# Ham3798/shielded-pool-pinocchio-solana

Hardware: AMD Instinct MI355X
Metric: Groth16 proofs/sec (higher is better)
Workload: dtype u32x8 (254-bit Montgomery integers); 1 GPU; audit_circuit (RLWE, const-PK; scripts/generate_audit.py:246-465), batch of 2048 independent proofs per GPU per step, every row a distinct witness; circuit=audit, n_constraints=29178, n_wires=35432, domain=32768, batch_per_gpu=2048, n_distinct_witnesses=2048, table_bytes=226725433344, parallelism=independent proofs x1, pk_bytes=9850060

## Files before the change

shielded-pool-pinocchio-solana_amd/csrc/bn254_consts.hpp:

```cpp
#pragma once
#include <stdint.h>
namespace spp {
struct FrParams {
  static constexpr uint32_t MOD(int i) { constexpr uint32_t v[8] = {0xf0000001u, 0x43e1f593u, 0x79b97091u, 0x2833e848u, 0x8181585du, 0xb85045b6u, 0xe131a029u, 0x30644e72u}; return v[i]; }
  static constexpr uint32_t ONE(int i) { constexpr uint32_t v[8] = {0x4ffffffbu, 0xac96341cu, 0x9f60cd29u, 0x36fc7695u, 0x7879462eu, 0x666ea36fu, 0x9a07df2fu, 0x0e0a77c1u}; return v[i]; }
  static constexpr uint32_t R2(int i) { constexpr uint32_t v[8] = {0xae216da7u, 0x1bb8e645u, 0xe35c59e3u, 0x53fe3ab1u, 0x53bb8085u, 0x8c49833du, 0x7f4e44a5u, 0x0216d0b1u}; return v[i]; }
  static constexpr uint32_t R3(int i) { constexpr uint32_t v[8] = {0xb4bf0040u, 0x5e94d8e1u, 0x1cfbb6b8u, 0x2a489cbeu, 0xa19fcfedu, 0x893cc664u, 0x7fcc657cu, 0x0cf8594bu}; return v[i]; }
  static constexpr uint32_t HALF(int i) { constexpr uint32_t v[8] = {0xf8000000u, 0xa1f0fac9u, 0x3cdcb848u, 0x9419f424u, 0x40c0ac2eu, 0xdc2822dbu, 0x7098d014u, 0x18322739u}; return v[i]; }
  static constexpr uint32_t MODM2(int i) { constexpr uint32_t v[8] = {0xefffffffu, 0x43e1f593u, 0x79b97091u, 0x2833e848u, 0x8181585du, 0xb85045b6u, 0xe131a029u, 0x30644e72u}; return v[i]; }
  static constexpr uint32_t TWOP(int i) { constexpr uint32_t v[8] = {0xe0000002u, 0x87c3eb27u, 0xf372e122u, 0x5067d090u, 0x0302b0bau, 0x70a08b6du, 0xc2634053u, 0x60c89ce5u}; return v[i]; }
  static constexpr uint32_t INV32 = 0xefffffffu;
  static constexpr uint32_t K29_IN(int i) { constexpr uint32_t v[9] = {0x0fffead7u, 0x1d5444f4u, 0x04438aa5u, 0x03b4d096u, 0x134c84dau, 0x0e92d304u, 0x14cb95b3u, 0x041b9d3du, 0x00058003u}; return v[i]; }
  static constexpr uint32_t K29_ZZ_OUT(int i) { constexpr uint32_t v[9] = {0x00000000u, 0x00000000u, 0x00000000u, 0x00000000u, 0x00000000u, 0x00000000u, 0x00000000u, 0x00000000u, 0x00080000u}; return v[i]; }
  static constexpr uint32_t K29_ONE(int i) { constexpr uint32_t v[9] = {0x0fffff57u, 0x1ea70ab4u, 0x052c068bu, 0x17504f49u, 0x0aa8075bu, 0x1d4240ceu, 0x11d54c07u, 0x052ac7a8u, 0x000dc836u}; return v[i]; }
  static constexpr uint32_t SUBC_2P_1(int i) { constexpr uint32_t v[9] = {0x20000002u, 0x3e1f593eu, 0x3cb848a0u, 0x2fa121e5u, 0x2b0ba505u, 0x25b68180u, 0x214dc281u, 0x3cb84c67u, 0x0060c89bu}; return v[i]; }
  static constexpr uint32_t SUBC_4P_1(int i) { constexpr uint32_t v[9] = {0x20000004u, 0x3c3eb27du, 0x39709142u, 0x3f4243ccu, 0x36174a0bu, 0x2b6d0301u, 0x229b8503u, 0x397098cfu, 0x00c19138u}; return v[i]; }
  static constexpr uint32_t SUBC_6P_1(int i) { constexpr uint32_t v[9] = {0x20000006u, 0x3a5e0bbcu, 0x3628d9e4u, 0x2ee365b3u, 0x2122ef12u, 0x31238483u, 0x23e94785u, 0x3628e537u, 0x012259d5u}; return v[i]; }
  static constexpr uint32_t SUBC_8P_1(int i) { constexpr uint32_t v[9] = {0x20000008u, 0x387d64fbu, 0x32e12286u, 0x3e84879au, 0x2c2e9418u, 0x36da0604u, 0x25370a07u, 0x32e1319fu, 0x01832272u}; return v[i]; }
  static constexpr uint32_t SUBC_4P_3(int i) { constexpr uint32_t v[9] = {0x60000004u, 0x7c3eb27bu, 0x79709140u, 0x7f4243cau, 0x76174a09u, 0x6b6d02ffu, 0x629b8501u, 0x797098cdu, 0x00c19136u}; return v[i]; }
  static constexpr uint32_t SUBC_8P_3(int i) { constexpr uint32_t v[9] = {0x60000008u, 0x787d64f9u, 0x72e12284u, 0x7e848798u, 0x6c2e9416u, 0x76da0602u, 0x65370a05u, 0x72e1319du, 0x01832270u}; return v[i]; }
  static constexpr uint32_t SUBC_16P_3(int i) { constexpr uint32_t v[9] = {0x60000010u, 0x70fac9f5u, 0x65c2450cu, 0x7d090f34u, 0x785d2830u, 0x6db40c07u, 0x6a6e140eu, 0x65c2633du, 0x030644e4u}; return v[i]; }
};
struct FqParams {
  static constexpr uint32_t MOD(int i) { constexpr uint32_t v[8] = {0xd87cfd47u, 0x3c208c16u, 0x6871ca8du, 0x97816a91u, 0x8181585du, 0xb85045b6u, 0xe131a029u, 0x30644e72u}; return v[i]; }
  static constexpr uint32_t ONE(int i) { constexpr uint32_t v[8] = {0xc58f0d9du, 0xd35d438du, 0xf5c70b3du, 0x0a78eb28u, 0x7879462cu, 0x666ea36fu, 0x9a07df2fu, 0x0e0a77c1u}; return v[i]; }
  static constexpr uint32_t R2(int i) { constexpr uint32_t v[8] = {0x538afa89u, 0xf32cfc5bu, 0xd44501fbu, 0xb5e71911u, 0x0a417ff6u, 0x47ab1effu, 0xcab8351fu, 0x06d89f71u}; return v[i]; }
  static constexpr uint32_t R3(int i) { constexpr uint32_t v[8] = {0xda1530dfu, 0xb1cd6dafu, 0xa7283db6u, 0x62f210e6u, 0x0ada0afbu, 0xef7f0b0cu, 0x2d592544u, 0x20fd6e90u}; return v[i]; }
  static constexpr uint32_t HALF(int i) { constexpr uint32_t v[8] = {0x6c3e7ea3u, 0x9e10460bu, 0xb438e546u, 0xcbc0b548u, 0x40c0ac2eu, 0xdc2822dbu, 0x7098d014u, 0x18322739u}; return v[i]; }
  static constexpr uint32_t MODM2(int i) { constexpr uint32_t v[8] = {0xd87cfd45u, 0x3c208c16u, 0x6871ca8du, 0x97816a91u, 0x8181585du, 0xb85045b6u, 0xe131a029u, 0x30644e72u}; return v[i]; }
  static constexpr uint32_t TWOP(int i) { constexpr uint32_t v[8] = {0xb0f9fa8eu, 0x7841182du, 0xd0e3951au, 0x2f02d522u, 0x0302b0bbu, 0x70a08b6du, 0xc2634053u, 0x60c89ce5u}; return v[i]; }
  static constexpr uint32_t INV32 = 0xe4866389u;
  static constexpr uint32_t K29_IN(int i) { constexpr uint32_t v[9] = {0x13349ca1u, 0x1a5d84a8u, 0x0a3e5cacu, 0x100249e0u, 0x12b951e8u, 0x0e92d304u, 0x14cb95b3u, 0x041b9d3du, 0x00058003u}; return v[i]; }
  static constexpr uint32_t K29_ZZ_OUT(int i) { constexpr uint32_t v[9] = {0x00000000u, 0x00000000u, 0x00000000u, 0x00000000u, 0x00000000u, 0x00000000u, 0x00000000u, 0x00000000u, 0x00080000u}; return v[i]; }
  static constexpr uint32_t K29_ONE(int i) { constexpr uint32_t v[9] = {0x157ccc21u, 0x141c2758u, 0x185230d3u, 0x014c0419u, 0x0aa36fb9u, 0x1d4240ceu, 0x11d54c07u, 0x052ac7a8u, 0x000dc836u}; return v[i]; }
  static constexpr uint32_t SUBC_2P_1(int i) { constexpr uint32_t v[9] = {0x30f9fa8eu, 0x2208c16cu, 0x38e5469du, 0x25aa45a0u, 0x2b0bb2efu, 0x25b68180u, 0x214dc281u, 0x3cb84c67u, 0x0060c89bu}; return v[i]; }
  static constexpr uint32_t SUBC_4P_1(int i) { constexpr uint32_t v[9] = {0x21f3f51cu, 0x241182dau, 0x31ca8d3bu, 0x2b548b42u, 0x361765dfu, 0x2b6d0301u, 0x229b8503u, 0x397098cfu, 0x00c19138u}; return v[i]; }
  static constexpr uint32_t SUBC_6P_1(int i) { constexpr uint32_t v[9] = {0x32edefaau, 0x261a4447u, 0x2aafd3d9u, 0x30fed0e4u, 0x212318cfu, 0x31238483u, 0x23e94785u, 0x3628e537u, 0x012259d5u}; return v[i]; }
  static constexpr uint32_t SUBC_8P_1(int i) { constexpr uint32_t v[9] = {0x23e7ea38u, 0x282305b5u, 0x23951a77u, 0x36a91686u, 0x2c2ecbbfu, 0x36da0604u, 0x25370a07u, 0x32e1319fu, 0x01832272u}; return v[i]; }
  static constexpr uint32_t SUBC_4P_3(int i) { constexpr uint32_t v[9] = {0x61f3f51cu, 0x641182d8u, 0x71ca8d39u, 0x6b548b40u, 0x761765ddu, 0x6b6d02ffu, 0x629b8501u, 0x797098cdu, 0x00c19136u}; return v[i]; }
  static constexpr uint32_t SUBC_8P_3(int i) { constexpr uint32_t v[9] = {0x63e7ea38u, 0x682305b3u, 0x63951a75u, 0x76a91684u, 0x6c2ecbbdu, 0x76da0602u, 0x65370a05u, 0x72e1319du, 0x01832270u}; return v[i]; }
  static constexpr uint32_t SUBC_16P_3(int i) { constexpr uint32_t v[9] = {0x67cfd470u, 0x70460b69u, 0x672a34edu, 0x6d522d0bu, 0x785d977eu, 0x6db40c07u, 0x6a6e140eu, 0x65c2633du, 0x030644e4u}; return v[i]; }
};
}
```

shielded-pool-pinocchio-solana_amd/csrc/f29.hpp:

```cpp
#pragma once
#include "bn254.hpp"

#if defined(__HIPCC__)
#define SPP_HD_COLD __host__ __device__ __attribute__((noinline))
#else
#define SPP_HD_COLD __attribute__((noinline))
#endif

namespace spp {

template <class Pm>
struct F29 {
  uint32_t l[9];
  using Base = Fp<Pm>;
  typedef uint32_t (*ConstFn)(int);
  static constexpr uint32_t M = (1u << 29) - 1u;
  static constexpr uint32_t INV = Pm::INV32 & M;
  static SPP_HD constexpr uint32_t P9(int k) { return Base::P9(k); }

  template <ConstFn C>
  static SPP_HD F29 konst() {
    F29 r;
    SPP_UNROLL for (int i = 0; i < 9; i++) r.l[i] = C(i);
    return r;
// ... 62 lines not shown
  }
  SPP_HD F29 sqr() const {
    uint64_t c[18];
    clear(c);
    mac_sqr(c, *this);
    return reduce(c);
  }
  static SPP_HD F29 mul2(const F29& a, const F29& b, const F29& cc, const F29& d) {
    uint64_t c[18];
    clear(c);
    mac(c, a, b);
    mac(c, cc, d);
    return reduce(c);
  }

  template <ConstFn C>
  static SPP_HD F29 sub_lazy(const F29& a, const F29& b) {
    F29 r;
    SPP_UNROLL for (int k = 0; k < 9; k++) r.l[k] = a.l[k] + (C(k) - b.l[k]);
    return r;
  }
  template <ConstFn C>
  static SPP_HD F29 neg_lazy(const F29& b) {
    F29 r;
    SPP_UNROLL for (int k = 0; k < 9; k++) r.l[k] = C(k) - b.l[k];
    return r;
  }
  template <ConstFn C>
  static SPP_HD F29 sub_norm(const F29& a, const F29& b) {
    F29 r;
// ... 25 lines not shown
  }
  friend SPP_HD F29 add_norm(const F29& a, const F29& b) {
    F29 r;
    uint32_t carry = 0;
    SPP_UNROLL for (int k = 0; k < 8; k++) {
      const uint32_t t = a.l[k] + b.l[k] + carry;
      r.l[k] = t & M;
      carry = t >> 29;
    }
    r.l[8] = a.l[8] + b.l[8] + carry;
    return r;
  }

  template <uint32_t KMAX>
  SPP_HD bool is_zero_mod_p() const {
    uint32_t kk = 0xffffffffu;
    SPP_UNROLL for (uint32_t k = 0; k <= KMAX; k++) {
      if (l[0] == ((k * P9(0)) & M)) kk = k;
    }
    if (kk == 0xffffffffu) return false;
    uint32_t diff = 0, carry = 0;
    SPP_UNROLL for (int i = 0; i < 8; i++) {
      const uint32_t t = kk * P9(i) + carry;
      diff |= l[i] ^ (t & M);
      carry = t >> 29;
    }
    diff |= l[8] ^ (kk * P9(8) + carry);
    return diff == 0;
  }

  static SPP_HD F29 from_fp(const Base& a) { return from_words(a.l) * konst<Pm::K29_IN>(); }
  SPP_HD Base to_fp() const {
    uint32_t w[8];
    SPP_UNROLL for (int i = 0; i < 8; i++) w[i] = Pm::ONE(i);
    const F29 t = *this * from_words(w);
    Base r;
    t.to_words(r.l);
    return r;
  }
  SPP_HD Base scaled_to_fp() const {
    const F29 t = *this * konst<Pm::K29_ZZ_OUT>();
    Base r;
    t.to_words(r.l);
    return r;
  }
};

template <class Pm>
struct XYZZ29 {
  using F = F29<Pm>;
  using B = Fp<Pm>;
  F X, Y, ZZ, ZZZ;
  bool inf;

  static SPP_HD XYZZ29 infinity() {
    XYZZ29 r;
    SPP_UNROLL for (int i = 0; i < 9; i++) r.X.l[i] = r.Y.l[i] = r.ZZ.l[i] = r.ZZZ.l[i] = 0;
    r.inf = true;
    return r;
  }
  SPP_HD XYZZ<B> to_xyzz() const {
    if (inf) return XYZZ<B>::infinity();
    return {X.to_fp(), Y.to_fp(), ZZ.scaled_to_fp(), ZZZ.scaled_to_fp()};
// ... 11 lines not shown
  SPP_HD void madd(const Affine<B>& e, bool negate) { madd_any<false>(e, negate); }
  SPP_HD bool madd_distinct(const Affine<B>& e, bool negate) { return madd_any<true>(e, negate); }
  template <bool DISTINCT>
  SPP_HD bool madd_any(const Affine<B>& e, bool negate) {
    F x2 = F::from_words(e.x.l);
    F y2 = F::from_words(e.y.l);
    if (negate) y2 = F::template neg_lazy<Pm::SUBC_4P_1>(y2);
    if (inf) {
      X = x2 * F::template konst<Pm::K29_IN>();
      Y = y2 * F::template konst<Pm::K29_IN>();
      ZZ = F::template konst<Pm::K29_IN>();
      ZZZ = ZZ;
      inf = false;
      return true;
    }
    const F U2 = x2 * ZZ;
    const F Pp = F::template sub_norm<Pm::SUBC_6P_1>(U2, X);
    if (Pp.template is_zero_mod_p<7>()) {
      if constexpr (DISTINCT) return false;
      const F S2 = y2 * ZZZ;
      const F Rr = F::template sub_norm<Pm::SUBC_2P_1>(S2, Y);
      if (Rr.template is_zero_mod_p<3>()) {
        XYZZ<B> t = to_xyzz();
        t.dbl_inplace();
        const XYZZ29 d = from_xyzz(t);
        X = d.X;
        Y = d.Y;
        ZZ = d.ZZ;
        ZZZ = d.ZZZ;
      } else {
        inf = true;
      }
      return true;
    }
    const F PP = Pp.sqr();
    const F Q = X * PP;
    const F PPP = Pp * PP;
    ZZ = ZZ * PP;
    const F S2 = y2 * ZZZ;
    const F Rr = F::template sub_norm<Pm::SUBC_2P_1>(S2, Y);
    ZZZ = ZZZ * PPP;
    const F R2 = Rr.sqr();
    X = F::template sub3_norm<Pm::SUBC_4P_3>(R2, PPP, Q);
    const F T = F::template sub_lazy<Pm::SUBC_6P_1>(Q, X);
    const F Yn = F::template neg_lazy<Pm::SUBC_2P_1>(Y);
    Y = F::mul2(Rr, T, Yn, PPP);
    return true;
  }
};

struct F29x2 {
  using F = F29<FqParams>;
  using Pm = FqParams;
  F c0, c1;

  static SPP_HD F29x2 from_words(const Fq2& a) { return {F::from_words(a.c0.l), F::from_words(a.c1.l)}; }
  template <F::ConstFn CA>
  static SPP_HD F29x2 mul(const F29x2& a, const F29x2& b) {
    const F na1 = F::template neg_lazy<CA>(a.c1);
    return {F::mul2(a.c0, b.c0, na1, b.c1), F::mul2(a.c0, b.c1, a.c1, b.c0)};
  }
  SPP_HD F29x2 mul_real(const F& k) const { return {c0 * k, c1 * k}; }
  template <F::ConstFn CA>
  SPP_HD F29x2 sqr() const {
    const F s = add_lazy(c0, c1);
    const F d = F::template sub_lazy<CA>(c0, c1);
    const F t = add_lazy(c0, c0);
    return {s * d, t * c1};
  }
  template <F::ConstFn C>
  static SPP_HD F29x2 sub_norm(const F29x2& a, const F29x2& b) {
    return {F::template sub_norm<C>(a.c0, b.c0), F::template sub_norm<C>(a.c1, b.c1)};
  }
  template <F::ConstFn C>
  static SPP_HD F29x2 sub3_norm(const F29x2& a, const F29x2& b, const F29x2& c2) {
    return {F::template sub3_norm<C>(a.c0, b.c0, c2.c0), F::template sub3_norm<C>(a.c1, b.c1, c2.c1)};
  }
  template <F::ConstFn C>
  static SPP_HD F29x2 neg_lazy(const F29x2& a) {
    return {F::template neg_lazy<C>(a.c0), F::template neg_lazy<C>(a.c1)};
  }
  template <uint32_t KMAX>
  SPP_HD bool is_zero_mod_p() const {
    return c0.template is_zero_mod_p<KMAX>() && c1.template is_zero_mod_p<KMAX>();
  }
  SPP_HD Fq2 to_fp() const { return {c0.to_fp(), c1.to_fp()}; }
  SPP_HD Fq2 scaled_to_fp() const { return {c0.scaled_to_fp(), c1.scaled_to_fp()}; }
  static SPP_HD F29x2 from_fp(const Fq2& a) { return {F::from_fp(a.c0), F::from_fp(a.c1)}; }
};

struct XYZZ29G2 {
  using E = F29x2;
  using F = F29<FqParams>;
  using Pm = FqParams;
  E X, Y, ZZ, ZZZ;
  bool inf;

  static SPP_HD XYZZ29G2 infinity() {
    XYZZ29G2 r;
    SPP_UNROLL for (int i = 0; i < 9; i++) {
      r.X.c0.l[i] = r.X.c1.l[i] = r.Y.c0.l[i] = r.Y.c1.l[i] = 0;
      r.ZZ.c0.l[i] = r.ZZ.c1.l[i] = r.ZZZ.c0.l[i] = r.ZZZ.c1.l[i] = 0;
    }
    r.inf = true;
    return r;
  }
  SPP_HD XYZZ<Fq2> to_xyzz() const {
    if (inf) return XYZZ<Fq2>::infinity();
    return {X.to_fp(), Y.to_fp(), ZZ.scaled_to_fp(), ZZZ.scaled_to_fp()};
  }
  static SPP_HD XYZZ29G2 from_xyzz(const XYZZ<Fq2>& q) {
    XYZZ29G2 r;
    r.inf = q.is_inf();
    const F k = F::template konst<Pm::K29_IN>();
    r.X = E::from_fp(q.X);
    r.Y = E::from_fp(q.Y);
    r.ZZ = E::from_fp(q.ZZ).mul_real(k);
    r.ZZZ = E::from_fp(q.ZZZ).mul_real(k);
    return r;
  }

  SPP_HD void madd(const Affine<Fq2>& e, bool negate) { madd_any<false>(e, negate); }
  SPP_HD bool madd_distinct(const Affine<Fq2>& e, bool negate) { return madd_any<true>(e, negate); }
  template <bool DISTINCT>
  SPP_HD bool madd_any(const Affine<Fq2>& e, bool negate) {
    const E x2 = E::from_words(e.x);
    const E y2 = E::from_words(e.y);
// ... 3 lines not shown
      const E yn = E::template neg_lazy<Pm::SUBC_4P_1>(y2);
      E ys;
      SPP_UNROLL for (int i = 0; i < 9; i++) {
        ys.c0.l[i] = negate ? yn.c0.l[i] : y2.c0.l[i];
        ys.c1.l[i] = negate ? yn.c1.l[i] : y2.c1.l[i];
      }
      Y = ys.mul_real(k);
      SPP_UNROLL for (int i = 0; i < 9; i++) {
        ZZ.c0.l[i] = k.l[i];
        ZZ.c1.l[i] = 0;
      }
      ZZZ = ZZ;
      inf = false;
      return true;
    }
    const E U2 = E::template mul<Pm::SUBC_4P_1>(x2, ZZ);
    const E Pp = E::template sub_norm<Pm::SUBC_6P_1>(U2, X);
    E S2 = E::template mul<Pm::SUBC_4P_1>(y2, ZZZ);
    if (negate) S2 = E::template neg_lazy<Pm::SUBC_2P_1>(S2);
    const E Rr = E::template sub_norm<Pm::SUBC_2P_1>(S2, Y);
    if (Pp.template is_zero_mod_p<7>()) {
      if constexpr (DISTINCT) return false;
      if (Rr.template is_zero_mod_p<4>()) {
        XYZZ<Fq2> t = to_xyzz();
        t.dbl_inplace();
        const XYZZ29G2 d = from_xyzz(t);
        X = d.X;
        Y = d.Y;
        ZZ = d.ZZ;
        ZZZ = d.ZZZ;
      } else {
        inf = true;
      }
      return true;
    }
    const E PP = Pp.template sqr<Pm::SUBC_8P_1>();
    const E Q = E::template mul<Pm::SUBC_6P_1>(X, PP);
    const E PPP = E::template mul<Pm::SUBC_8P_1>(Pp, PP);
    ZZ = E::template mul<Pm::SUBC_2P_1>(ZZ, PP);
    ZZZ = E::template mul<Pm::SUBC_2P_1>(ZZZ, PPP);
    const E R2 = Rr.template sqr<Pm::SUBC_6P_1>();
    X = E::template sub3_norm<Pm::SUBC_4P_3>(R2, PPP, Q);
    const E T = E::template sub_norm<Pm::SUBC_6P_1>(Q, X);
    const F nR1 = F::template neg_lazy<Pm::SUBC_6P_1>(Rr.c1);
    const F nY0 = F::template neg_lazy<Pm::SUBC_2P_1>(Y.c0);
    const F nY1 = F::template neg_lazy<Pm::SUBC_2P_1>(Y.c1);
    uint64_t c[18];
    F::clear(c);
    F::mac(c, Rr.c0, T.c0);
    F::mac(c, nR1, T.c1);
    F::mac(c, nY0, PPP.c0);
    F::mac(c, Y.c1, PPP.c1);
    const F y0 = F::reduce(c);
    F::clear(c);
    F::mac(c, Rr.c0, T.c1);
    F::mac(c, Rr.c1, T.c0);
    F::mac(c, nY0, PPP.c1);
    F::mac(c, nY1, PPP.c0);
    Y.c0 = y0;
    Y.c1 = F::reduce(c);
    return true;
  }
};

}
```

shielded-pool-pinocchio-solana_amd/csrc/gen_consts.py:

```python
#!/usr/bin/env python3
R_MOD = 21888242871839275222246405745257275088548364400416034343698204186575808495617
Q_MOD = 21888242871839275222246405745257275088696311157297823662689037894645226208583


def limbs(v):
    return ", ".join("0x%08xu" % ((v >> (32 * i)) & 0xFFFFFFFF) for i in range(8))


def limbs29(v):
    return ", ".join("0x%08xu" % ((v >> (29 * i)) & ((1 << 29) - 1) if i < 8 else v >> 232) for i in range(9))


def lifted(m, k, lowmin):
    v = k * m
    c = [(v >> (29 * i)) & ((1 << 29) - 1) for i in range(8)] + [v >> 232]
    for i in range(8):
        while c[i] < lowmin:
            c[i] += 1 << 29
            c[i + 1] -= 1
    assert c[8] > 0 and sum(x << (29 * i) for i, x in enumerate(c)) == v and all(x < (1 << 32) for x in c)
    return c


def emit(name, m):
    W = 1 << 256
    inv32 = (-pow(m, -1, 1 << 32)) % (1 << 32)
    out = []
    out.append("struct %s {" % name)
    for cname, val in (("MOD", m), ("ONE", W % m), ("R2", W * W % m), ("R3", W * W * W % m),
                       ("HALF", (m - 1) // 2), ("MODM2", m - 2), ("TWOP", 2 * m)):
        out.append("  static constexpr uint32_t %s(int i) { constexpr uint32_t v[8] = {%s}; return v[i]; }"
                   % (cname, limbs(val)))
    out.append("  static constexpr uint32_t INV32 = 0x%08xu;" % inv32)
    W9 = 1 << 261
    for cname, val in (("K29_IN", W9 * W9 * pow(W, -1, m) % m),
                       ("K29_ZZ_OUT", W * W * pow(W9, -1, m) % m),
                       ("K29_ONE", W9 % m)):
        out.append("  static constexpr uint32_t %s(int i) { constexpr uint32_t v[9] = {%s}; return v[i]; }"
                   % (cname, limbs29(val)))
    for k, low in ((2, 1), (4, 1), (6, 1), (8, 1), (4, 3), (8, 3), (16, 3)):
        out.append("  static constexpr uint32_t SUBC_%dP_%d(int i) { constexpr uint32_t v[9] = {%s}; return v[i]; }"
                   % (k, low, ", ".join("0x%08xu" % x for x in lifted(m, k, low * ((1 << 29) - 1)))))
    out.append("};")
    return "\n".join(out)


print("// AUTO-GENERATED by gen_consts.py -- do not edit.")
print("#pragma once\n#include <stdint.h>\nnamespace spp {")
# ... 4 lines not shown
```

shielded-pool-pinocchio-solana_amd/csrc/kernels.hpp:

```cpp
#pragma once
#include <hip/hip_runtime.h>
#include <stdint.h>
#include "bn254.hpp"
#include "msm_plan.hpp"
#include "msm_ragged.hpp"
#include "rlwe_ntt.hpp"

namespace spp {

struct DevSparse {
  const uint32_t* rowptr;
  const uint32_t* wire;
  const uint32_t* coeff;
  const uint32_t* lit;
};
static constexpr uint32_t COEFF_ONE = 0x80000000u;
static constexpr uint32_t COEFF_MINUS_ONE = 0x40000000u;
static constexpr uint32_t COEFF_MASK = 0x3fffffffu;

struct HashConsts {
  const Fr* pos3_rc;  const Fr* pos3_mds;
  const Fr* pos5_rc;  const Fr* pos5_mds;
  const Fr* p2_rc;    const Fr* p2_mu;
  const uint32_t* pos3_mds29;
// ... 134 lines not shown
                         const int32_t* prov, const int32_t* proof_ok, int32_t dup, int32_t* result);
void launch_pool_commit(hipStream_t st, const PoolSet& set, uint64_t salt, const uint8_t* keys, uint32_t stride, uint32_t count, const int32_t* result,
                        uint32_t* set_count);
void launch_spmv_check(hipStream_t st, DevCircuit dc, const Fr* W, Fr* abc, uint32_t n, uint32_t P, uint32_t* status, int16_t* small = nullptr);

void launch_ntt(hipStream_t st, Fr* data, uint32_t logn, uint32_t P, const Fr* tw, bool dif, uint32_t nbatch, size_t batch_stride,
                const Fr* post = nullptr);
void launch_scale_rows(hipStream_t st, Fr* data, const Fr* table, uint32_t n, uint32_t P, uint32_t nbatch, size_t batch_stride);
void launch_qap_pointwise(hipStream_t st, Fr* abc, uint32_t n, uint32_t P, Fr zinv);
void launch_qap_product(hipStream_t st, Fr* abc, uint32_t n, uint32_t P);

template <class F>
struct MsmWalk;
template <>
struct MsmWalk<Fq> {
  static constexpr uint32_t waves_per_simd = 2;
  static constexpr uint32_t rows_waves_per_simd = 2;
  static constexpr bool gather_ahead = false;
  static constexpr uint32_t occ(uint32_t Wt) { return Wt == 1 ? waves_per_simd : rows_waves_per_simd; }
};
template <>
struct MsmWalk<Fq2> {
  static constexpr uint32_t waves_per_simd = 2;
  static constexpr uint32_t rows_waves_per_simd = 1;
  static constexpr bool gather_ahead = false;
  static constexpr uint32_t occ(uint32_t Wt) { return Wt == 1 ? waves_per_simd : rows_waves_per_simd; }
};
template <class F>
void launch_build_table(hipStream_t st, const Affine<F>* bases, uint32_t N, uint32_t c, uint32_t Wt, uint32_t row0, uint32_t nrows,
                        Affine<F>* table, XYZZ<F>* tmp, F* tmp_pre, const MsmBlock* blocks = nullptr, uint32_t E = 0);
void launch_msm_digits(hipStream_t st, const uint32_t* rows, const Fr* scalars, int16_t* dig, uint32_t N, uint32_t P, uint32_t c);
template <class F>
void launch_msm_accumulate(hipStream_t st, const Affine<F>* table, const MsmBlock* blocks, const int16_t* dig, XYZZ<F>* partial, uint32_t N, uint32_t P,
                           uint32_t c, const MsmPlan& pl, hipEvent_t ev_start = nullptr, hipEvent_t ev_stop = nullptr, uint32_t* redo_count = nullptr);
template <class F>
void launch_msm_reduce(hipStream_t st, XYZZ<F>* partial, XYZZ<F>* out, uint32_t P, const MsmPlan& pl, uint32_t c, bool empty);
static constexpr uint32_t MSM_FOLD_SETS = 8;
static constexpr uint32_t MSM_FOLD_RADIX = 8;
template <class F>
struct MsmFoldSets {
// ... 45 lines not shown
```

shielded-pool-pinocchio-solana_amd/csrc/msm_table.hpp:

```cpp
#pragma once
#include <hip/hip_ext.h>
#include "kernels.hpp"
#include <algorithm>
#include "f29.hpp"

namespace spp {

static constexpr unsigned MSM_FOLD_COOP_MAX_BATCH = 8;
static constexpr unsigned MSM_WALK_BLOCK = 64;

template <class F>
__global__ void __launch_bounds__(64) k_build_table(const Affine<F>* __restrict__ bases, uint32_t N, uint32_t E, uint32_t Wn,
                                                    uint32_t step_bits, uint32_t row0, uint32_t nrows, Affine<F>* __restrict__ table,
                                                    XYZZ<F>* __restrict__ tmp, F* __restrict__ tmp_pre, const MsmBlock* __restrict__ blocks) {
  const uint32_t rl = blockIdx.x * blockDim.x + threadIdx.x;
  if (rl >= nrows) return;
  const uint32_t row = row0 + rl;
  const size_t off = blocks ? (size_t)blocks[row >> 6].off : (size_t)(row >> 6) * E;
  Affine<F>* out = table + off * 64 + (row & 63);
  XYZZ<F>* t = tmp + rl;
  F* pre = tmp_pre + rl;
  if (row >= N * Wn) {
    for (uint32_t d = 0; d < E; d++) out[(size_t)d * 64] = Affine<F>::infinity();
    return;
// ... 61 lines not shown
      carry = 1;
      sgn = !neg;
    } else {
      carry = 0;
      sgn = neg;
    }
    return d;
  }
};

__device__ __forceinline__ bool words_all_zero(const Fq& v) {
  uint32_t o = 0;
  SPP_UNROLL for (int i = 0; i < 8; i++) o |= v.l[i];
  return o == 0;
}
template <class F>
struct MsmAcc;
template <>
struct MsmAcc<Fq> {
  XYZZ29<FqParams> a;
  __device__ __forceinline__ void init() { a = XYZZ29<FqParams>::infinity(); }
  __device__ __forceinline__ void madd(const Affine<Fq>& e, bool sgn) {
    if (words_all_zero(e.x) && words_all_zero(e.y)) return;
    a.madd(e, sgn);
  }
  __device__ __forceinline__ bool madd_distinct(const Affine<Fq>& e, bool sgn) {
    if (words_all_zero(e.x) && words_all_zero(e.y)) return true;
    return a.madd_distinct(e, sgn);
  }
  __device__ __forceinline__ XYZZ<Fq> result() const { return a.to_xyzz(); }
};

template <>
struct MsmAcc<Fq2> {
  XYZZ29G2 a;
  __device__ __forceinline__ void init() { a = XYZZ29G2::infinity(); }
  __device__ __forceinline__ void madd(const Affine<Fq2>& e, bool sgn) {
    if (words_all_zero(e.x.c0) && words_all_zero(e.x.c1) && words_all_zero(e.y.c0) && words_all_zero(e.y.c1)) return;
    a.madd(e, sgn);
  }
  __device__ __forceinline__ bool madd_distinct(const Affine<Fq2>& e, bool sgn) {
    if (words_all_zero(e.x.c0) && words_all_zero(e.x.c1) && words_all_zero(e.y.c0) && words_all_zero(e.y.c1)) return true;
    return a.madd_distinct(e, sgn);
  }
  __device__ __forceinline__ XYZZ<Fq2> result() const { return a.to_xyzz(); }
};


template <class F>
__device__ __forceinline__ void msm_store_redo_marker(XYZZ<F>* out) {
  static_assert(sizeof(XYZZ<F>) % 16 == 0, "stored as 16-byte words");
  uint4* w = reinterpret_cast<uint4*>(out);
  SPP_UNROLL for (uint32_t i = 0; i < sizeof(XYZZ<F>) / 16; i++) w[i] = make_uint4(0, 0, 0, 0);
}
template <class F>
__device__ __forceinline__ bool msm_is_redo_marker(const XYZZ<F>* v) {
  const uint32_t* x = reinterpret_cast<const uint32_t*>(&v->X);
  const uint32_t* zz = reinterpret_cast<const uint32_t*>(&v->ZZ);
  uint32_t o = 0;
  SPP_UNROLL for (uint32_t i = 0; i < sizeof(F) / 4; i++) o |= x[i] | zz[i];
  return o == 0;
}
template <class F, bool FAST>
__device__ __forceinline__ bool msm_flat_walk(MsmAcc<F>& acc, const Affine<F>* __restrict__ table, const MsmBlock* __restrict__ blocks,
                                              const int16_t* __restrict__ dg, uint32_t N, uint32_t Pp, uint32_t sl, uint32_t Sg) {
  if constexpr (FAST && MsmWalk<F>::gather_ahead) {
    int d_next = 0;
    Affine<F> e_next;
    for (uint32_t i0 = sl;; i0 += 4 * Sg) {
      const bool last = i0 >= N;
      uint64_t pack = 0;
      if (!last) {
        SPP_UNROLL for (uint32_t k = 0; k < 4; k++) {
          const uint32_t i = i0 + k * Sg;
          const uint32_t d = i < N ? (uint32_t)(uint16_t)dg[(size_t)i * Pp] : 0u;
          pack |= (uint64_t)d << (16 * k);
        }
      }
#pragma unroll 1
// ... 41 lines not shown
          }
        }
      }
    }
  }
  return true;
}
template <class F>
__global__ void __launch_bounds__(MSM_WALK_BLOCK, MsmWalk<F>::waves_per_simd) k_msm_flat(const Affine<F>* __restrict__ table, const MsmBlock* __restrict__ blocks,
                                                  const int16_t* __restrict__ dig, XYZZ<F>* __restrict__ partial, uint32_t N, uint32_t P,
                                                  uint32_t Pp, uint32_t R, uint32_t Sg) {
  const uint32_t g = blockIdx.x * blockDim.x + threadIdx.x;
  const uint32_t p = g % Pp, t = g / Pp;
  if (t >= R * Sg || p >= P) return;
  const uint32_t rho = t / Sg, sl = t % Sg;
  MsmAcc<F> acc;
  acc.init();
  if (msm_flat_walk<F, true>(acc, table, blocks, dig + ((size_t)rho * N) * Pp + p, N, Pp, sl, Sg)) partial[(size_t)t * P + p] = acc.result();
  else msm_store_redo_marker(partial + (size_t)t * P + p);
}
template <class F>
__global__ void __launch_bounds__(MSM_WALK_BLOCK, MsmWalk<F>::waves_per_simd) k_msm_flat_redo(const Affine<F>* __restrict__ table, const MsmBlock* __restrict__ blocks,
                                                  const int16_t* __restrict__ dig, XYZZ<F>* __restrict__ partial, uint32_t N, uint32_t P,
                                                  uint32_t Pp, uint32_t R, uint32_t Sg, uint32_t* __restrict__ redo_count) {
  const uint32_t g = blockIdx.x * blockDim.x + threadIdx.x;
  const uint32_t p = g % Pp, t = g / Pp;
  if (t >= R * Sg || p >= P) return;
  XYZZ<F>* out = partial + (size_t)t * P + p;
  if (!msm_is_redo_marker(out)) return;
  if (redo_count) atomicAdd(redo_count, 1u);
  const uint32_t rho = t / Sg, sl = t % Sg;
// ... 229 lines not shown
```

Baseline: 7090 proofs/s.

## Add product-scanning Montgomery forms for F29 and raise G1 MSM walk occupancy

Adds an operand-scanning-by-column Montgomery multiply (Scan) that keeps a single 64-bit accumulator and interleaves reduction per column. An optional opaque barrier forces serial accumulation, and a paired variant interleaves two independent products. The G1 flat MSM walk now uses the serial scan form and launches with 3 waves per SIMD instead of 2, aiming to cut register pressure and raise occupancy. is_zero_mod_p now uses a modular inverse of p mod 2^29 instead of a search loop. The risk is a longer dependent chain per multiply and possible spills under the tighter register budget.

```diff
diff --git a/profiles/f29_scan_accounting.py b/profiles/f29_scan_accounting.py
--- /dev/null
+++ b/profiles/f29_scan_accounting.py
@@ -0,0 +1,88 @@
+#!/usr/bin/env python3
+import re
+import sys
+
+KERNELS = ("k_msm_flat", "k_msm_flat_redo")
+
+
+def kernels(text):
+    out = {}
+    lines = text.split("\n")
+    i = 0
+    while i < len(lines):
+        m = re.match(r"^(_ZN3spp\w+):\s*(;.*)?$", lines[i])
+        if m:
+            j = i + 1
+            while j < len(lines) and "s_endpgm" not in lines[j]:
+                j += 1
+            k = j
+            res = {}
+            while k < len(lines) and k < j + 80:
+                for key, pat in (("vgpr", r"; NumVgprs: (\d+)"), ("agpr", r"; NumAgprs: (\d+)"), ("scratch", r"; ScratchSize: (\d+)"),
+                                 ("occ", r"; Occupancy: (\d+)")):
+                    mm = re.match(pat, lines[k])
+                    if mm and key not in res:
+                        res[key] = int(mm.group(1))
+                k += 1
+            out[m.group(1)] = (lines[i + 1:j], res)
+            i = j
+        i += 1
+    return out
+
+
+def loop_blocks(body, whole=False):
+    blocks = [("", [], [])]
+    for line in body:
+        s = line.strip()
+        m = re.match(r"^(\.LBB\w+):", s)
+        if m:
+            blocks.append((m.group(1), [], []))
+        elif s and not s.startswith((".", ";")) and not s.split()[0].endswith(":"):
+            blocks[-1][1].append(s.split()[0])
+            if s.startswith(("s_cbranch", "s_branch")):
+                blocks[-1][2].append(s.split()[1])
+    index = {b[0]: n for n, b in enumerate(blocks)}
+    inside = set()
+    for n, (_, _, targets) in enumerate(blocks):
+        for t in targets:
+            if t in index and index[t] <= n:
+                inside.update(range(index[t], n + 1))
+    if whole:
+        inside = set(range(len(blocks)))
+    return [blocks[n][1] for n in sorted(inside)]
+
+
+def pretty(sym):
+    for name in sorted(KERNELS, key=len, reverse=True):
+        tag = "%d%sI" % (len(name), name)
+        if tag in sym:
+            field = "Fq2" if "Fp2" in sym or "Fq2" in sym else "Fq"
+            return "%s<%s>" % (name, field)
+    return None
+
+
+def main():
+    print("%-8s %-24s %6s %6s %6s %6s %6s %5s %5s %8s %5s" % ("commit", "kernel", "instr", "mad64", "add64", "shr64", "s_nop", "VGPR", "AGPR", "scratch", "waves"))
+    for arg in sys.argv[1:]:
+        label, path = arg.split(":", 1)
+        for sym, (body, res) in sorted(kernels(open(path).read()).items()):
+            name = pretty(sym)
+            if not name:
+                continue
+            tot = mad = add = shr = nop = 0
+            chosen = [b for b in loop_blocks(body) if b.count("v_mad_u64_u32") >= 100]
+            if not chosen:
+                chosen = [b for b in loop_blocks(body + ["s_branch .LBB_all"], whole=True) if b.count("v_mad_u64_u32") >= 100]
+                name += " *"
+            for b in chosen:
+                tot += len(b)
+                mad += b.count("v_mad_u64_u32")
+                add += b.count("v_lshl_add_u64") + sum(1 for op in b if op.startswith("v_addc_co_u32"))
+                shr += b.count("v_lshrrev_b64")
+                nop += b.count("s_nop")
+            print("%-8s %-24s %6d %6d %6d %6d %6d %5s %5s %8s %5s" % (label, name, tot, mad, add, shr, nop, res.get("vgpr"), res.get("agpr"),
+                                                                   res.get("scratch"), res.get("occ")))
+
+
+if __name__ == "__main__":
+    main()
diff --git a/shielded-pool-pinocchio-solana_amd/csrc/bn254_consts.hpp b/shielded-pool-pinocchio-solana_amd/csrc/bn254_consts.hpp
--- a/shielded-pool-pinocchio-solana_amd/csrc/bn254_consts.hpp
+++ b/shielded-pool-pinocchio-solana_amd/csrc/bn254_consts.hpp
@@ -10,6 +10,7 @@
   static constexpr uint32_t MODM2(int i) { constexpr uint32_t v[8] = {0xefffffffu, 0x43e1f593u, 0x79b97091u, 0x2833e848u, 0x8181585du, 0xb85045b6u, 0xe131a029u, 0x30644e72u}; return v[i]; }
   static constexpr uint32_t TWOP(int i) { constexpr uint32_t v[8] = {0xe0000002u, 0x87c3eb27u, 0xf372e122u, 0x5067d090u, 0x0302b0bau, 0x70a08b6du, 0xc2634053u, 0x60c89ce5u}; return v[i]; }
   static constexpr uint32_t INV32 = 0xefffffffu;
+  static constexpr uint32_t PINV29 = 0x10000001u;
   static constexpr uint32_t K29_IN(int i) { constexpr uint32_t v[9] = {0x0fffead7u, 0x1d5444f4u, 0x04438aa5u, 0x03b4d096u, 0x134c84dau, 0x0e92d304u, 0x14cb95b3u, 0x041b9d3du, 0x00058003u}; return v[i]; }
   static constexpr uint32_t K29_ZZ_OUT(int i) { constexpr uint32_t v[9] = {0x00000000u, 0x00000000u, 0x00000000u, 0x00000000u, 0x00000000u, 0x00000000u, 0x00000000u, 0x00000000u, 0x00080000u}; return v[i]; }
   static constexpr uint32_t K29_ONE(int i) { constexpr uint32_t v[9] = {0x0fffff57u, 0x1ea70ab4u, 0x052c068bu, 0x17504f49u, 0x0aa8075bu, 0x1d4240ceu, 0x11d54c07u, 0x052ac7a8u, 0x000dc836u}; return v[i]; }
@@ -30,6 +31,7 @@
   static constexpr uint32_t MODM2(int i) { constexpr uint32_t v[8] = {0xd87cfd45u, 0x3c208c16u, 0x6871ca8du, 0x97816a91u, 0x8181585du, 0xb85045b6u, 0xe131a029u, 0x30644e72u}; return v[i]; }
   static constexpr uint32_t TWOP(int i) { constexpr uint32_t v[8] = {0xb0f9fa8eu, 0x7841182du, 0xd0e3951au, 0x2f02d522u, 0x0302b0bbu, 0x70a08b6du, 0xc2634053u, 0x60c89ce5u}; return v[i]; }
   static constexpr uint32_t INV32 = 0xe4866389u;
+  static constexpr uint32_t PINV29 = 0x1b799c77u;
   static constexpr uint32_t K29_IN(int i) { constexpr uint32_t v[9] = {0x13349ca1u, 0x1a5d84a8u, 0x0a3e5cacu, 0x100249e0u, 0x12b951e8u, 0x0e92d304u, 0x14cb95b3u, 0x041b9d3du, 0x00058003u}; return v[i]; }
   static constexpr uint32_t K29_ZZ_OUT(int i) { constexpr uint32_t v[9] = {0x00000000u, 0x00000000u, 0x00000000u, 0x00000000u, 0x00000000u, 0x00000000u, 0x00000000u, 0x00000000u, 0x00080000u}; return v[i]; }
   static constexpr uint32_t K29_ONE(int i) { constexpr uint32_t v[9] = {0x157ccc21u, 0x141c2758u, 0x185230d3u, 0x014c0419u, 0x0aa36fb9u, 0x1d4240ceu, 0x11d54c07u, 0x052ac7a8u, 0x000dc836u}; return v[i]; }
diff --git a/shielded-pool-pinocchio-solana_amd/csrc/f29.hpp b/shielded-pool-pinocchio-solana_amd/csrc/f29.hpp
--- a/shielded-pool-pinocchio-solana_amd/csrc/f29.hpp
+++ b/shielded-pool-pinocchio-solana_amd/csrc/f29.hpp
@@ -7,7 +7,15 @@
 #define SPP_HD_COLD __attribute__((noinline))
 #endif
 
+#if defined(__HIP_DEVICE_COMPILE__)
+#define SPP_OPAQUE(x) asm("" : "+v"(x))
+#else
+#define SPP_OPAQUE(x) ((void)0)
+#endif
+
 namespace spp {
+
+enum F29Form : int { F29_COLUMNS = 0, F29_SCAN_CARRY = 1, F29_SCAN_SERIAL = 2, F29_SCAN_PAIRS = 3 };
 
 template <class Pm>
 struct F29 {
@@ -100,6 +108,147 @@
     return reduce(c);
   }
 
+  template <bool SERIAL>
+  struct Scan {
+    uint64_t acc = 0;
+    uint32_t m[9];
+    F29 r;
+    SPP_HD void fma(uint32_t x, uint32_t y) {
+      acc += (uint64_t)x * y;
+      if constexpr (SERIAL) SPP_OPAQUE(acc);
+    }
+    SPP_HD void ab(int k, int i, const F29& a, const F29& b) {
+      const int j = k - i;
+      if (j >= 0 && j < 9) fma(a.l[i], b.l[j]);
+    }
+    SPP_HD void sq(int k, int i, const F29& a, const uint32_t (&d)[9]) {
+      const int j = k - i;
+      if (j == i) fma(a.l[i], a.l[i]);
+      else if (j > i && j < 9) fma(a.l[i], d[j]);
+    }
+    SPP_HD void mp(int k, int i) {
+      const int j = k - i;
+      if (i < k && j >= 0 && j < 9) fma(m[i], P9(j));
+    }
+    SPP_HD void end(int k) {
+      if (k < 9) {
+        m[k] = ((uint32_t)acc * INV) & M;
+        fma(m[k], P9(0));
+      } else {
+        r.l[k - 9] = (uint32_t)acc & M;
+      }
+      acc >>= 29;
+      SPP_OPAQUE(acc);
+      if (k == 16) r.l[8] = (uint32_t)acc;
+    }
+  };
+  template <bool SERIAL, int NP>
+  static SPP_HD F29 dot_scan(const F29* const (&a)[NP], const F29* const (&b)[NP]) {
+    Scan<SERIAL> s;
+    SPP_UNROLL for (int k = 0; k < 17; k++) {
+      SPP_UNROLL for (int t = 0; t < NP; t++) {
+        SPP_UNROLL for (int i = 0; i < 9; i++) s.ab(k, i, *a[t], *b[t]);
+      }
+      SPP_UNROLL for (int i = 0; i < 9; i++) s.mp(k, i);
+      s.end(k);
+    }
+    return s.r;
+  }
+  template <bool SERIAL>
+  SPP_HD F29 sqr_scan() const {
+    uint32_t d[9];
+    SPP_UNROLL for (int i = 0; i < 9; i++) d[i] = l[i] << 1;
+    Scan<SERIAL> s;
+    SPP_UNROLL for (int k = 0; k < 17; k++) {
+      SPP_UNROLL for (int i = 0; i < 9; i++) s.sq(k, i, *this, d);
+      SPP_UNROLL for (int i = 0; i < 9; i++) s.mp(k, i);
+      s.end(k);
+    }
+    return s.r;
+  }
+  template <int NP0, int NP1>
+  static SPP_HD void dot_scan_pair(F29& r0, const F29* const (&a0)[NP0], const F29* const (&b0)[NP0], F29& r1, const F29* const (&a1)[NP1],
+                                   const F29* const (&b1)[NP1]) {
+    Scan<true> s0, s1;
+    SPP_UNROLL for (int k = 0; k < 17; k++) {
+      SPP_UNROLL for (int t = 0; t < (NP0 > NP1 ? NP0 : NP1); t++) {
+        SPP_UNROLL for (int i = 0; i < 9; i++) {
+          if (t < NP0) s0.ab(k, i, *a0[t < NP0 ? t : 0], *b0[t < NP0 ? t : 0]);
+          if (t < NP1) s1.ab(k, i, *a1[t < NP1 ? t : 0], *b1[t < NP1 ? t : 0]);
+        }
+      }
+      SPP_UNROLL for (int i = 0; i < 9; i++) {
+        s0.mp(k, i);
+        s1.mp(k, i);
+      }
+      s0.end(k);
+      s1.end(k);
+    }
+    r0 = s0.r;
+    r1 = s1.r;
+  }
+  static SPP_HD void sqr_scan_pair(F29& r0, const F29& a0, F29& r1, const F29& a1) {
+    uint32_t d0[9], d1[9];
+    SPP_UNROLL for (int i = 0; i < 9; i++) {
+      d0[i] = a0.l[i] << 1;
+      d1[i] = a1.l[i] << 1;
+    }
+    Scan<true> s0, s1;
+    SPP_UNROLL for (int k = 0; k < 17; k++) {
+      SPP_UNROLL for (int i = 0; i < 9; i++) {
+        s0.sq(k, i, a0, d0);
+        s1.sq(k, i, a1, d1);
+      }
+      SPP_UNROLL for (int i = 0; i < 9; i++) {
+        s0.mp(k, i);
+        s1.mp(k, i);
+      }
+      s0.end(k);
+      s1.end(k);
+    }
+    r0 = s0.r;
+    r1 = s1.r;
+  }
+  static SPP_HD void mul_scan_pair(F29& r0, const F29& a0, const F29& b0, F29& r1, const F29& a1, const F29& b1) {
+    const F29* const x0[1] = {&a0};
+    const F29* const y0[1] = {&b0};
+    const F29* const x1[1] = {&a1};
+    const F29* const y1[1] = {&b1};
+    dot_scan_pair<1, 1>(r0, x0, y0, r1, x1, y1);
+  }
+  template <int FORM>
+  static SPP_HD F29 mul_as(const F29& a, const F29& b) {
+    if constexpr (FORM == F29_COLUMNS) return a * b;
+    else {
+      const F29* const x[1] = {&a};
+      const F29* const y[1] = {&b};
+      return dot_scan<(FORM >= F29_SCAN_SERIAL), 1>(x, y);
+    }
+  }
+  template <int FORM>
+  SPP_HD F29 sqr_as() const {
+    if constexpr (FORM == F29_COLUMNS) return sqr();
+    else return sqr_scan<(FORM >= F29_SCAN_SERIAL)>();
+  }
+  template <int FORM>
+  static SPP_HD F29 mul2_as(const F29& a, const F29& b, const F29& cc, const F29& d) {
+    if constexpr (FORM == F29_COLUMNS) return mul2(a, b, cc, d);
+    else {
+      const F29* const x[2] = {&a, &cc};
+      const F29* const y[2] = {&b, &d};
+      return dot_scan<(FORM >= F29_SCAN_SERIAL), 2>(x, y);
+    }
+  }
+  template <int FORM>
+  static SPP_HD F29 mul4_as(const F29* const (&a)[4], const F29* const (&b)[4]) {
+    if constexpr (FORM == F29_COLUMNS) {
+      uint64_t c[18];
+      clear(c);
+      SPP_UNROLL for (int t = 0; t < 4; t++) mac(c, *a[t], *b[t]);
+      return reduce(c);
+    } else return dot_scan<(FORM >= F29_SCAN_SERIAL), 4>(a, b);
+  }
+
   template <ConstFn C>
   static SPP_HD F29 sub_lazy(const F29& a, const F29& b) {
     F29 r;
@@ -155,11 +304,8 @@
 
   template <uint32_t KMAX>
   SPP_HD bool is_zero_mod_p() const {
-    uint32_t kk = 0xffffffffu;
-    SPP_UNROLL for (uint32_t k = 0; k <= KMAX; k++) {
-      if (l[0] == ((k * P9(0)) & M)) kk = k;
-    }
-    if (kk == 0xffffffffu) return false;
+    const uint32_t kk = (l[0] * Pm::PINV29) & M;
+    if (kk > KMAX) return false;
     uint32_t diff = 0, carry = 0;
     SPP_UNROLL for (int i = 0; i < 8; i++) {
       const uint32_t t = kk * P9(i) + carry;
@@ -187,7 +333,7 @@
   }
 };
 
-template <class Pm>
+template <class Pm, int FORM = F29_COLUMNS>
 struct XYZZ29 {
   using F = F29<Pm>;
   using B = Fp<Pm>;
@@ -229,38 +375,65 @@
       inf = false;
       return true;
     }
-    const F U2 = x2 * ZZ;
+    if constexpr (FORM == F29_SCAN_PAIRS) {
+      F U2, S2;
+      F::mul_scan_pair(U2, x2, ZZ, S2, y2, ZZZ);
+      const F Pp = F::template sub_norm<Pm::SUBC_6P_1>(U2, X);
+      const F Rr = F::template sub_norm<Pm::SUBC_2P_1>(S2, Y);
+      if (Pp.template is_zero_mod_p<7>()) {
+        if constexpr (DISTINCT) return false;
+        same_x(Rr);
+        return true;
+      }
+      F PP, R2;
+      F::sqr_scan_pair(PP, Pp, R2, Rr);
+      F Q, PPP;
+      F::mul_scan_pair(Q, X, PP, PPP, Pp, PP);
+      ZZ = F::template mul_as<FORM>(ZZ, PP);
+      X = F::template sub3_norm<Pm::SUBC_4P_3>(R2, PPP, Q);
+      const F T = F::template sub_lazy<Pm::SUBC_6P_1>(Q, X);
+      const F Yn = F::template neg_lazy<Pm::SUBC_2P_1>(Y);
+      const F* const za[1] = {&ZZZ};
+      const F* const zb[1] = {&PPP};
+      const F* const ya[2] = {&Rr, &Yn};
+      const F* const yb[2] = {&T, &PPP};
+      F::template dot_scan_pair<1, 2>(ZZZ, za, zb, Y, ya, yb);
+      return true;
+    }
+    const F U2 = F::template mul_as<FORM>(x2, ZZ);
     const F Pp = F::template sub_norm<Pm::SUBC_6P_1>(U2, X);
     if (Pp.template is_zero_mod_p<7>()) {
       if constexpr (DISTINCT) return false;
-      const F S2 = y2 * ZZZ;
-      const F Rr = F::template sub_norm<Pm::SUBC_2P_1>(S2, Y);
-      if (Rr.template is_zero_mod_p<3>()) {
-        XYZZ<B> t = to_xyzz();
-        t.dbl_inplace();
-        const XYZZ29 d = from_xyzz(t);
-        X = d.X;
-        Y = d.Y;
-        ZZ = d.ZZ;
-        ZZZ = d.ZZZ;
-      } else {
-        inf = true;
-      }
+      const F S2 = F::template mul_as<FORM>(y2, ZZZ);
+      same_x(F::template sub_norm<Pm::SUBC_2P_1>(S2, Y));
       return true;
     }
-    const F PP = Pp.sqr();
-    const F Q = X * PP;
-    const F PPP = Pp * PP;
-    ZZ = ZZ * PP;
-    const F S2 = y2 * ZZZ;
+    const F PP = Pp.template sqr_as<FORM>();
+    const F Q = F::template mul_as<FORM>(X, PP);
+    const F PPP = F::template mul_as<FORM>(Pp, PP);
+    ZZ = F::template mul_as<FORM>(ZZ, PP);
+    const F S2 = F::template mul_as<FORM>(y2, ZZZ);
     const F Rr = F::template sub_norm<Pm::SUBC_2P_1>(S2, Y);
-    ZZZ = ZZZ * PPP;
-    const F R2 = Rr.sqr();
+    ZZZ = F::template mul_as<FORM>(ZZZ, PPP);
+    const F R2 = Rr.template sqr_as<FORM>();
     X = F::template sub3_norm<Pm::SUBC_4P_3>(R2, PPP, Q);
     const F T = F::template sub_lazy<Pm::SUBC_6P_1>(Q, X);
     const F Yn = F::template neg_lazy<Pm::SUBC_2P_1>(Y);
-    Y = F::mul2(Rr, T, Yn, PPP);
+    Y = F::template mul2_as<FORM>(Rr, T, Yn, PPP);
     return true;
+  }
+  SPP_HD void same_x(const F& Rr) {
+    if (Rr.template is_zero_mod_p<3>()) {
+      XYZZ<B> t = to_xyzz();
+      t.dbl_inplace();
+      const XYZZ29 d = from_xyzz(t);
+      X = d.X;
+      Y = d.Y;
+      ZZ = d.ZZ;
+      ZZZ = d.ZZZ;
+    } else {
+      inf = true;
+    }
   }
 };
 
@@ -270,18 +443,30 @@
   F c0, c1;
 
   static SPP_HD F29x2 from_words(const Fq2& a) { return {F::from_words(a.c0.l), F::from_words(a.c1.l)}; }
-  template <F::ConstFn CA>
+  template <F::ConstFn CA, int FORM = F29_COLUMNS>
   static SPP_HD F29x2 mul(const F29x2& a, const F29x2& b) {
     const F na1 = F::template neg_lazy<CA>(a.c1);
-    return {F::mul2(a.c0, b.c0, na1, b.c1), F::mul2(a.c0, b.c1, a.c1, b.c0)};
+    if constexpr (FORM == F29_SCAN_PAIRS) {
+      const F* const xa[2] = {&a.c0, &na1};
+      const F* const xb[2] = {&b.c0, &b.c1};
+      const F* const ya[2] = {&a.c0, &a.c1};
+      const F* const yb[2] = {&b.c1, &b.c0};
+      F29x2 r;
+      F::template dot_scan_pair<2, 2>(r.c0, xa, xb, r.c1, ya, yb);
+      return r;
+    } else return {F::template mul2_as<FORM>(a.c0, b.c0, na1, b.c1), F::template mul2_as<FORM>(a.c0, b.c1, a.c1, b.c0)};
   }
   SPP_HD F29x2 mul_real(const F& k) const { return {c0 * k, c1 * k}; }
-  template <F::ConstFn CA>
+  template <F::ConstFn CA, int FORM = F29_COLUMNS>
   SPP_HD F29x2 sqr() const {
     const F s = add_lazy(c0, c1);
     const F d = F::template sub_lazy<CA>(c0, c1);
     const F t = add_lazy(c0, c0);
-    return {s * d, t * c1};
+    if constexpr (FORM == F29_SCAN_PAIRS) {
+      F29x2 r;
+      F::mul_scan_pair(r.c0, s, d, r.c1, t, c1);
+      return r;
+    } else return {F::template mul_as<FORM>(s, d), F::template mul_as<FORM>(t, c1)};
   }
   template <F::ConstFn C>
   static SPP_HD F29x2 sub_norm(const F29x2& a, const F29x2& b) {
@@ -304,15 +489,16 @@
   static SPP_HD F29x2 from_fp(const Fq2& a) { return {F::from_fp(a.c0), F::from_fp(a.c1)}; }
 };
 
-struct XYZZ29G2 {
+template <int FORM>
+struct XYZZ29G2F {
   using E = F29x2;
   using F = F29<FqParams>;
   using Pm = FqParams;
   E X, Y, ZZ, ZZZ;
   bool inf;
 
-  static SPP_HD XYZZ29G2 infinity() {
-    XYZZ29G2 r;
+  static SPP_HD XYZZ29G2F infinity() {
+    XYZZ29G2F r;
     SPP_UNROLL for (int i = 0; i < 9; i++) {
       r.X.c0.l[i] = r.X.c1.l[i] = r.Y.c0.l[i] = r.Y.c1.l[i] = 0;
       r.ZZ.c0.l[i] = r.ZZ.c1.l[i] = r.ZZZ.c0.l[i] = r.ZZZ.c1.l[i] = 0;
@@ -324,8 +510,8 @@
     if (inf) return XYZZ<Fq2>::infinity();
     return {X.to_fp(), Y.to_fp(), ZZ.scaled_to_fp(), ZZZ.scaled_to_fp()};
   }
-  static SPP_HD XYZZ29G2 from_xyzz(const XYZZ<Fq2>& q) {
-    XYZZ29G2 r;
+  static SPP_HD XYZZ29G2F from_xyzz(const XYZZ<Fq2>& q) {
+    XYZZ29G2F r;
     r.inf = q.is_inf();
     const F k = F::template konst<Pm::K29_IN>();
     r.X = E::from_fp(q.X);
@@ -359,9 +545,9 @@
       inf = false;
       return true;
     }
-    const E U2 = E::template mul<Pm::SUBC_4P_1>(x2, ZZ);
+    const E U2 = E::template mul<Pm::SUBC_4P_1, FORM>(x2, ZZ);
     const E Pp = E::template sub_norm<Pm::SUBC_6P_1>(U2, X);
-    E S2 = E::template mul<Pm::SUBC_4P_1>(y2, ZZZ);
+    E S2 = E::template mul<Pm::SUBC_4P_1, FORM>(y2, ZZZ);
     if (negate) S2 = E::template neg_lazy<Pm::SUBC_2P_1>(S2);
     const E Rr = E::template sub_norm<Pm::SUBC_2P_1>(S2, Y);
     if (Pp.template is_zero_mod_p<7>()) {
@@ -369,7 +555,7 @@
       if (Rr.template is_zero_mod_p<4>()) {
         XYZZ<Fq2> t = to_xyzz();
         t.dbl_inplace();
-        const XYZZ29G2 d = from_xyzz(t);
+        const XYZZ29G2F d = from_xyzz(t);
         X = d.X;
         Y = d.Y;
         ZZ = d.ZZ;
@@ -379,33 +565,31 @@
       }
       return true;
     }
-    const E PP = Pp.template sqr<Pm::SUBC_8P_1>();
-    const E Q = E::template mul<Pm::SUBC_6P_1>(X, PP);
-    const E PPP = E::template mul<Pm::SUBC_8P_1>(Pp, PP);
-    ZZ = E::template mul<Pm::SUBC_2P_1>(ZZ, PP);
-    ZZZ = E::template mul<Pm::SUBC_2P_1>(ZZZ, PPP);
-    const E R2 = Rr.template sqr<Pm::SUBC_6P_1>();
+    const E PP = Pp.template sqr<Pm::SUBC_8P_1, FORM>();
+    const E Q = E::template mul<Pm::SUBC_6P_1, FORM>(X, PP);
+    const E PPP = E::template mul<Pm::SUBC_8P_1, FORM>(Pp, PP);
+    ZZ = E::template mul<Pm::SUBC_2P_1, FORM>(ZZ, PP);
+    ZZZ = E::template mul<Pm::SUBC_2P_1, FORM>(ZZZ, PPP);
+    const E R2 = Rr.template sqr<Pm::SUBC_6P_1, FORM>();
     X = E::template sub3_norm<Pm::SUBC_4P_3>(R2, PPP, Q);
     const E T = E::template sub_norm<Pm::SUBC_6P_1>(Q, X);
     const F nR1 = F::template neg_lazy<Pm::SUBC_6P_1>(Rr.c1);
     const F nY0 = F::template neg_lazy<Pm::SUBC_2P_1>(Y.c0);
     const F nY1 = F::template neg_lazy<Pm::SUBC_2P_1>(Y.c1);
-    uint64_t c[18];
-    F::clear(c);
-    F::mac(c, Rr.c0, T.c0);
-    F::mac(c, nR1, T.c1);
-    F::mac(c, nY0, PPP.c0);
-    F::mac(c, Y.c1, PPP.c1);
-    const F y0 = F::reduce(c);
-    F::clear(c);
-    F::mac(c, Rr.c0, T.c1);
-    F::mac(c, Rr.c1, T.c0);
-    F::mac(c, nY0, PPP.c1);
-    F::mac(c, nY1, PPP.c0);
-    Y.c0 = y0;
-    Y.c1 = F::reduce(c);
+    const F* const a0[4] = {&Rr.c0, &nR1, &nY0, &Y.c1};
+    const F* const b0[4] = {&T.c0, &T.c1, &PPP.c0, &PPP.c1};
+    const F* const a1[4] = {&Rr.c0, &Rr.c1, &nY0, &nY1};
+    const F* const b1[4] = {&T.c1, &T.c0, &PPP.c1, &PPP.c0};
+    if constexpr (FORM == F29_SCAN_PAIRS) {
+      F::template dot_scan_pair<4, 4>(Y.c0, a0, b0, Y.c1, a1, b1);
+    } else {
+      const F y0 = F::template mul4_as<FORM>(a0, b0);
+      Y.c1 = F::template mul4_as<FORM>(a1, b1);
+      Y.c0 = y0;
+    }
     return true;
   }
 };
+using XYZZ29G2 = XYZZ29G2F<F29_COLUMNS>;
 
 }
diff --git a/shielded-pool-pinocchio-solana_amd/csrc/gen_consts.py b/shielded-pool-pinocchio-solana_amd/csrc/gen_consts.py
--- a/shielded-pool-pinocchio-solana_amd/csrc/gen_consts.py
+++ b/shielded-pool-pinocchio-solana_amd/csrc/gen_consts.py
@@ -32,6 +32,7 @@
         out.append("  static constexpr uint32_t %s(int i) { constexpr uint32_t v[8] = {%s}; return v[i]; }"
                    % (cname, limbs(val)))
     out.append("  static constexpr uint32_t INV32 = 0x%08xu;" % inv32)
+    out.append("  static constexpr uint32_t PINV29 = 0x%08xu;" % pow(m, -1, 1 << 29))
     W9 = 1 << 261
     for cname, val in (("K29_IN", W9 * W9 * pow(W, -1, m) % m),
                        ("K29_ZZ_OUT", W * W * pow(W9, -1, m) % m),
diff --git a/shielded-pool-pinocchio-solana_amd/csrc/kernels.hpp b/shielded-pool-pinocchio-solana_amd/csrc/kernels.hpp
--- a/shielded-pool-pinocchio-solana_amd/csrc/kernels.hpp
+++ b/shielded-pool-pinocchio-solana_amd/csrc/kernels.hpp
@@ -2,6 +2,7 @@
 #include <hip/hip_runtime.h>
 #include <stdint.h>
 #include "bn254.hpp"
+#include "f29.hpp"
 #include "msm_plan.hpp"
 #include "msm_ragged.hpp"
 #include "rlwe_ntt.hpp"
@@ -172,9 +173,10 @@
 struct MsmWalk;
 template <>
 struct MsmWalk<Fq> {
-  static constexpr uint32_t waves_per_simd = 2;
+  static constexpr uint32_t waves_per_simd = 3;
   static constexpr uint32_t rows_waves_per_simd = 2;
   static constexpr bool gather_ahead = false;
+  static constexpr int product_form = F29_SCAN_SERIAL;
   static constexpr uint32_t occ(uint32_t Wt) { return Wt == 1 ? waves_per_simd : rows_waves_per_simd; }
 };
 template <>
@@ -182,6 +184,7 @@
   static constexpr uint32_t waves_per_simd = 2;
   static constexpr uint32_t rows_waves_per_simd = 1;
   static constexpr bool gather_ahead = false;
+  static constexpr int product_form = F29_COLUMNS;
   static constexpr uint32_t occ(uint32_t Wt) { return Wt == 1 ? waves_per_simd : rows_waves_per_simd; }
 };
 template <class F>
diff --git a/shielded-pool-pinocchio-solana_amd/csrc/msm_table.hpp b/shielded-pool-pinocchio-solana_amd/csrc/msm_table.hpp
--- a/shielded-pool-pinocchio-solana_amd/csrc/msm_table.hpp
+++ b/shielded-pool-pinocchio-solana_amd/csrc/msm_table.hpp
@@ -99,12 +99,12 @@
   SPP_UNROLL for (int i = 0; i < 8; i++) o |= v.l[i];
   return o == 0;
 }
-template <class F>
+template <class F, int FORM = F29_COLUMNS>
 struct MsmAcc;
-template <>
-struct MsmAcc<Fq> {
-  XYZZ29<FqParams> a;
-  __device__ __forceinline__ void init() { a = XYZZ29<FqParams>::infinity(); }
+template <int FORM>
+struct MsmAcc<Fq, FORM> {
+  XYZZ29<FqParams, FORM> a;
+  __device__ __forceinline__ void init() { a = XYZZ29<FqParams, FORM>::infinity(); }
   __device__ __forceinline__ void madd(const Affine<Fq>& e, bool sgn) {
     if (words_all_zero(e.x) && words_all_zero(e.y)) return;
     a.madd(e, sgn);
@@ -116,10 +116,10 @@
   __device__ __forceinline__ XYZZ<Fq> result() const { return a.to_xyzz(); }
 };
 
-template <>
-struct MsmAcc<Fq2> {
-  XYZZ29G2 a;
-  __device__ __forceinline__ void init() { a = XYZZ29G2::infinity(); }
+template <int FORM>
+struct MsmAcc<Fq2, FORM> {
+  XYZZ29G2F<FORM> a;
+  __device__ __forceinline__ void init() { a = XYZZ29G2F<FORM>::infinity(); }
   __device__ __forceinline__ void madd(const Affine<Fq2>& e, bool sgn) {
     if (words_all_zero(e.x.c0) && words_all_zero(e.x.c1) && words_all_zero(e.y.c0) && words_all_zero(e.y.c1)) return;
     a.madd(e, sgn);
@@ -146,8 +146,8 @@
   SPP_UNROLL for (uint32_t i = 0; i < sizeof(F) / 4; i++) o |= x[i] | zz[i];
   return o == 0;
 }
-template <class F, bool FAST>
-__device__ __forceinline__ bool msm_flat_walk(MsmAcc<F>& acc, const Affine<F>* __restrict__ table, const MsmBlock* __restrict__ blocks,
+template <class F, bool FAST, int FORM>
+__device__ __forceinline__ bool msm_flat_walk(MsmAcc<F, FORM>& acc, const Affine<F>* __restrict__ table, const MsmBlock* __restrict__ blocks,
                                               const int16_t* __restrict__ dg, uint32_t N, uint32_t Pp, uint32_t sl, uint32_t Sg) {
   if constexpr (FAST && MsmWalk<F>::gather_ahead) {
     int d_next = 0;
@@ -219,7 +219,7 @@
   const uint32_t p = g % Pp, t = g / Pp;
   if (t >= R * Sg || p >= P) return;
   const uint32_t rho = t / Sg, sl = t % Sg;
-  MsmAcc<F> acc;
+  MsmAcc<F, MsmWalk<F>::product_form> acc;
   acc.init();
   if (msm_flat_walk<F, true>(acc, table, blocks, dig + ((size_t)rho * N) * Pp + p, N, Pp, sl, Sg)) partial[(size_t)t * P + p] = acc.result();
   else msm_store_redo_marker(partial + (size_t)t * P + p);
```

Measured after the change: 7349 proofs/s (median of 6 runs). 1.04x the previous value.
